# haoxiangsnr/Wave-U-Net-for-Speech-Enhancement

Hardware: AMD Instinct MI355X
Metric: 16384-sample frames/sec fwd+bwd, 12-level Wave-U-Net (higher is better)
Workload: dtype f32 (levels >= 16 samples: 3 x f16 MFMA on hi/lo fp16 halves, fp32 accumulate; the rest f32 MFMA); 1 GPU; unet_basic 12-level, 16384-sample frames, batch=64 per GPU, fp32, training-mode forward + smooth_l1 + backward + fused HIP Adam step (BASELINE.json configs[2]; configs[3] when n_gpus>1); global_batch=64, frame=16384, parallelism=dp1

## Files before the change

wave-u-net-for-speech-enhancement_amd/csrc/wunet_h3u.h:

```cpp
#pragma once
#include "wunet_h3.h"
#ifndef WUNET_H3U_ABL
#define WUNET_H3U_ABL 0
#endif

struct ConvH3uArgs {
    const float* z0; const float* a0; const float* s0;
    const float* z1; const float* a1; const float* s1;
    const float* xb0; const float* xb1;
    float* xsc;
    float up_scale;
    int Lt;
    int C0, C1, C8;
    const wunet_half* wh; unsigned wdelta;
    const float* bias; const float* sc2;
    float* out; float* stats;
    const float* ev_a; const float* ev_s; float* xrows;
    wunet_half* oxh; wunet_half* oxl;
    int B, Cout, L, logL, NS, ntiles, mblocks;
    unsigned long long* trace;
};

__device__ __forceinline__ void wunet_h3u_x_scale(const float* xb0, const float* xb1, float& s, float& inv)
{
    wunet_pow2_scale(fmaxf(xb0[0], xb1 ? xb1[0] : 0.0f), s, inv);
}

#define WUNET_H3U_NST 8
__device__ __forceinline__ void wunet_loader_barrier(int younger)
{
#ifdef WUNET_EMU
    (void)younger;
    emu::block_barrier();
#else
    if (younger >= 10 + WUNET_H3U_NST) asm volatile("s_waitcnt vmcnt(18) lgkmcnt(0)\n\ts_barrier" ::: "memory");
    else if (younger >= 10) asm volatile("s_waitcnt vmcnt(10) lgkmcnt(0)\n\ts_barrier" ::: "memory");
    else if (younger == 9) asm volatile("s_waitcnt vmcnt(9) lgkmcnt(0)\n\ts_barrier" ::: "memory");
    else asm volatile("s_waitcnt vmcnt(0) lgkmcnt(0)\n\ts_barrier" ::: "memory");
    wunet_sched_fence();
#endif
}

__device__ __forceinline__ void wunet_loader_stats_barrier(int younger)
{
#ifdef WUNET_EMU
    (void)younger;
    emu::block_barrier();
#else
    if (younger >= 10 + WUNET_H3U_NST) asm volatile("s_waitcnt lgkmcnt(0) vmcnt(18)\n\ts_barrier" ::: "memory");
    else if (younger >= 10) asm volatile("s_waitcnt lgkmcnt(0) vmcnt(10)\n\ts_barrier" ::: "memory");
    else asm volatile("s_waitcnt lgkmcnt(0) vmcnt(0)\n\ts_barrier" ::: "memory");
    wunet_sched_fence();
#endif
}

struct WunetH3uRaw { wunet_f4 q[8]; float ma, mb; };
struct WunetH3uTile { int b, l0, mt0, ch; };
struct WunetH3uCursor { int ch, tile, mb; };
struct WunetH3uStep { int NS, mblocks, qG, rG; };
__device__ __forceinline__ void wunet_h3u_advance(WunetH3uCursor& c, const WunetH3uStep& S)
{
    if (++c.ch == S.NS) {
        c.ch = 0; c.tile += S.qG; c.mb += S.rG;
        if (c.mb >= S.mblocks) { c.mb -= S.mblocks; ++c.tile; }
    }
}
struct WunetH3uCoord { float w0[4], w1[4], mw0, mw1; };
__device__ __forceinline__ void wunet_h3u_coord(const ConvH3uArgs& A, int l0, int lane, WunetH3uCoord& K)
{
    const int Lth = A.Lt >> 1, P = l0 - 2 + 4 * lane;
#pragma unroll
    for (int j = 0; j < 4; ++j) {
        int i0, i1;
        wunet_up_coord(P + j < 0 ? 0 : P + j, Lth, A.up_scale, i0, i1, K.w0[j], K.w1[j]);
    }
    const int p_m = l0 + 254 + (lane & 3);
    int i0, i1;
    wunet_up_coord((lane < 32 && p_m < A.Lt) ? p_m : 0, Lth, A.up_scale, i0, i1, K.mw0, K.mw1);
}
__device__ __forceinline__ void wunet_h3u_mini_src(const ConvH3uArgs& A, int l0, int lane, int& i0, int& i1)
{
    const int p_m = l0 + 254 + (lane & 3);
    float w0, w1;
    wunet_up_coord((lane < 32 && p_m < A.Lt) ? p_m : 0, A.Lt >> 1, A.up_scale, i0, i1, w0, w1);
}

__device__ __forceinline__ unsigned long long wunet_sgpr64(unsigned long long b)
{
#ifdef WUNET_EMU
    return b;
#else
    const unsigned blo = __builtin_amdgcn_readfirstlane((unsigned)b), bhi = __builtin_amdgcn_readfirstlane((unsigned)(b >> 32));
    return ((unsigned long long)bhi << 32) | blo;
#endif
}
__device__ __forceinline__ wunet_f4 wunet_ld4s_async(unsigned long long sbase, unsigned voff)
{
#ifdef WUNET_EMU
    wunet_f4 v;
    std::memcpy(&v, reinterpret_cast<const char*>(sbase) + voff, 16);
    return v;
#else
    wunet_f4 v;
    asm volatile("global_load_dwordx4 %0, %1, %2" : "=v"(v) : "v"(voff), "s"(sbase) : "memory");
    return v;
#endif
}
__device__ __forceinline__ float wunet_ld1s_async(unsigned long long sbase, unsigned voff)
{
#ifdef WUNET_EMU
    float v;
    std::memcpy(&v, reinterpret_cast<const char*>(sbase) + voff, 4);
    return v;
#else
    float v;
    asm volatile("global_load_dword %0, %1, %2" : "=v"(v) : "v"(voff), "s"(sbase) : "memory");
    return v;
#endif
}
template <int N>
__device__ __forceinline__ void wunet_vm_wait()
{
#ifndef WUNET_EMU
    asm volatile("s_waitcnt vmcnt(%0)" :: "n"(N) : "memory");
    wunet_sched_fence();
#endif
}
__device__ __forceinline__ unsigned wunet_m0_save()
{
#ifdef WUNET_EMU
    return 0;
#else
    unsigned keep;
    asm volatile("s_mov_b32 %0, m0" : "=s"(keep) :: "memory");
    return keep;
#endif
}
__device__ __forceinline__ void wunet_m0_restore(unsigned keep)
{
#ifndef WUNET_EMU
    asm volatile("s_mov_b32 m0, %0" :: "s"(keep) : "memory");
#else
    (void)keep;
#endif
}
#ifdef WUNET_EMU
#define wunet_lds_uniform(X_) (X_)
#else
#define wunet_lds_uniform(X_) ((unsigned)__builtin_amdgcn_readfirstlane((int)(X_)))
#endif
template <int IMM>
__device__ __forceinline__ void wunet_dma16m(unsigned long long sbase, unsigned voff, wunet_lds_t lds_base)
{
#ifdef WUNET_EMU
    wunet_dma16(reinterpret_cast<const char*>(sbase) + voff, lds_base + IMM);
#else
    asm volatile("s_add_u32 m0, %2, %3\n\ts_nop 0\n\tglobal_load_lds_dwordx4 %0, %1" :: "v"(voff), "s"(sbase), "s"(lds_base), "n"(IMM) : "memory", "scc");
#endif
}

__device__ __forceinline__ int wunet_h3u_issue(const ConvH3uArgs& A, WunetH3uRaw& R, const WunetH3uTile& T, int cw, int lane, int mi0, int mi1)
{
    if (WUNET_H3U_ABL & 1) return 0;
    const int c8 = wunet_uniform(T.ch * 4 + cw);
    const int L = A.L, Lh = L >> 1, Lth = A.Lt >> 1;
    const bool none = c8 >= A.C8, up = !none && c8 * 8 < A.C0;
    const int P = T.l0 - 2 + 4 * lane;
    const int e_m = (lane >> 2) & 7, p_m = T.l0 + 254 + (lane & 3);
    const bool in_m = lane < 32 && p_m < A.Lt;
    int wb = (T.l0 >> 1) - 2 + 2 * lane;
    wb = wb < 0 ? 0 : (wb > Lth - 4 ? Lth - 4 : wb);
    const int pc = P < 0 ? 0 : (P > L - 4 ? L - 4 : P);
    const unsigned rs = none ? 0u : up ? (unsigned)Lh : (unsigned)L;
    const float* const zrow = up ? A.z0 + ((size_t)T.b * A.C0 + c8 * 8) * Lh : none ? A.z1 : A.z1 + ((size_t)T.b * A.C1 + (c8 * 8 - A.C0)) * L;
    unsigned long long rb = wunet_sgpr64((unsigned long long)(__UINTPTR_TYPE__)zrow);
    const unsigned long long rb0 = rb;
    const unsigned voff = none ? 0u : (unsigned)(up ? wb : pc) * 4u;
    const int m0 = up ? mi0 : (in_m ? p_m : 0), m1 = up ? mi1 : m0;
#pragma unroll
    for (int e = 0; e < 8; ++e) {
        R.q[e] = wunet_ld4s_async(rb, voff);
        rb = wunet_sgpr64(rb + (unsigned long long)rs * 4u);
    }
    R.ma = wunet_ld1s_async(rb0, none ? 0u : ((unsigned)e_m * rs + (unsigned)m0) * 4u);
    R.mb = wunet_ld1s_async(rb0, none ? 0u : ((unsigned)e_m * rs + (unsigned)m1) * 4u);
    return 10;
}

template <bool EDGE, bool COPY>
__device__ __forceinline__ void wunet_h3u_convert_t(const ConvH3uArgs& A, const WunetH3uRaw& R, const WunetH3uTile& T, wunet_half* xs, int cw,
                                                    int lane, const WunetH3uCoord& K, const float* coef, unsigned long long* tr)
{
#ifdef WUNET_H3U_TRACE
#define WUNET_H3U_SUB(K_) if (tr && cw == 0 && lane == 0) tr[K_] = wunet_memtime();
#else
#define WUNET_H3U_SUB(K_)
    (void)tr;
#endif
    WUNET_H3U_SUB(0)
    constexpr int COLS = 272, Q4 = COLS / 4;
    if (WUNET_H3U_ABL & 16) return;
    if (WUNET_H3U_ABL & 64) {
        float t = R.ma + R.mb;
#pragma unroll
        for (int e = 0; e < 8; ++e) t += R.q[e][0] + R.q[e][1] + R.q[e][2] + R.q[e][3];
        if (t == 123.456f) xs[lane] = 1;
        return;
    }
    const int c8 = wunet_uniform(T.ch * 4 + cw);
    const int L = A.L;
    const bool none = c8 >= A.C8, up = !none && c8 * 8 < A.C0;
    if (none) {
        const wunet_h8 z{0, 0, 0, 0, 0, 0, 0, 0};
#pragma unroll
        for (int j = 0; j < 4; ++j) {
            const int col = 4 * lane + 6 + j;
            const int pw = (cw * COLS + (col & 3) * Q4 + (col >> 2)) * 8;
            wunet_sth8(xs + pw, z);
            wunet_sth8(xs + 4 * COLS * 8 + pw, z);
        }
        if (lane < 32) {
            const int col = 262 + (lane & 3);
            const int pw = (cw * COLS + (col & 3) * Q4 + (col >> 2)) * 8 + (lane >> 2);
            xs[pw] = 0;
            xs[4 * COLS * 8 + pw] = 0;
        }
        return;
    }
    const bool write_out = COPY && T.mt0 == 0;
    const int cc = c8 * 8;
    float av[8], sv[8];
#pragma unroll
    for (int e = 0; e < 8; ++e) { av[e] = coef[cc + e]; sv[e] = coef[A.C8 * 8 + cc + e]; }
    WUNET_H3U_SUB(1)
    const int P = T.l0 - 2 + 4 * lane;
    const bool edge = EDGE && P < 0;
    float vals[4][8];
    if (up) {
#pragma unroll
        for (int e = 0; e < 8; ++e) {
            float u[4];
#pragma unroll
            for (int k = 0; k < 4; ++k) u[k] = wunet_lrelu(av[e] * R.q[e][k] + sv[e]);
            const float t0 = u[0], t1 = edge ? u[0] : u[1], t2 = edge ? u[0] : u[2], t3 = edge ? u[1] : u[3];
            vals[0][e] = K.w0[0] * t0 + K.w1[0] * t1;
            vals[1][e] = K.w0[1] * t1 + K.w1[1] * t2;
            vals[2][e] = K.w0[2] * t1 + K.w1[2] * t2;
            vals[3][e] = K.w0[3] * t2 + K.w1[3] * t3;
        }
    } else {
#pragma unroll
        for (int e = 0; e < 8; ++e) {
            float u[4];
#pragma unroll
            for (int k = 0; k < 4; ++k) u[k] = wunet_lrelu(av[e] * R.q[e][k] + sv[e]);
            vals[0][e] = u[0]; vals[1][e] = u[1];
            vals[2][e] = edge ? u[0] : u[2];
            vals[3][e] = edge ? u[1] : u[3];
        }
    }
    WUNET_H3U_SUB(2)
#pragma unroll
    for (int j = 0; j < 4; ++j) {
        wunet_h8 h, l;
#pragma unroll
        for (int e = 0; e < 8; ++e) {
            wunet_half x, y;
            wunet_split_h((edge && j < 2) ? 0.0f : vals[j][e], x, y);
            wunet_put_half(h, e, x);
            wunet_put_half(l, e, y);
        }
        const int col = 4 * lane + 6 + j;
        const int pw = (cw * COLS + (col & 3) * Q4 + (col >> 2)) * 8;
        if (!(WUNET_H3U_ABL & 128) || h[0] == (wunet_half)0x1234) {
        wunet_sth8(xs + pw, h);
        wunet_sth8(xs + 4 * COLS * 8 + pw, l);
        }
        if (write_out && col >= 8 && col < 264) {
            const size_t o = (((size_t)T.b * A.C8 + c8) * L + (size_t)(P + j)) * 8;
            wunet_sth8(A.oxh + o, h);
            wunet_sth8(A.oxl + o, l);
        }
    }
    WUNET_H3U_SUB(3)
    if (lane < 32) {
        const int e_m = lane >> 2, p_m = T.l0 + 254 + (lane & 3);
        const bool in_m = p_m < A.Lt;
        const float am = coef[cc + e_m], sm = coef[A.C8 * 8 + cc + e_m];
        const float ua = wunet_lrelu(am * R.ma + sm);
        const float v = up ? K.mw0 * ua + K.mw1 * wunet_lrelu(am * R.mb + sm) : ua;
        wunet_half x, y;
        wunet_split_h(in_m ? v : 0.0f, x, y);
        const int col = 262 + (lane & 3);
        const int pw = (cw * COLS + (col & 3) * Q4 + (col >> 2)) * 8 + e_m;
        xs[pw] = x;
        xs[4 * COLS * 8 + pw] = y;
        if (write_out && col < 264) {
            const size_t o = (((size_t)T.b * A.C8 + c8) * L + (size_t)p_m) * 8 + e_m;
            A.oxh[o] = x;
            A.oxl[o] = y;
        }
    }
#undef WUNET_H3U_SUB
}
template <bool COPY>
__device__ __forceinline__ void wunet_h3u_convert(const ConvH3uArgs& A, const WunetH3uRaw& R, const WunetH3uTile& T, wunet_half* xs, int cw,
                                                  int lane, const WunetH3uCoord& K, const float* coef, unsigned long long* tr = nullptr)
{
    if (wunet_uniform(T.l0) == 0) wunet_h3u_convert_t<true, COPY>(A, R, T, xs, cw, lane, K, coef, tr);
    else wunet_h3u_convert_t<false, COPY>(A, R, T, xs, cw, lane, K, coef, tr);
}

#ifdef WUNET_H3U_TRACE
#define WUNET_H3U_SUBPTR (A.trace && t < 128 ? A.trace + 256 * 2 * 128 * 2 + ((size_t)blockIdx.x * 128 + t) * 4 : nullptr)
#define WUNET_H3U_STAMP(ROLE_, STAGE_, WHICH_)                                                                     \
    if (A.trace && cw == 0 && lane == 0 && (STAGE_) < 128)                                                         \
        A.trace[(((size_t)blockIdx.x * 2 + (ROLE_)) * 128 + (STAGE_)) * 2 + (WHICH_)] = wunet_memtime();
#else
#define WUNET_H3U_SUBPTR nullptr
#define WUNET_H3U_STAMP(ROLE_, STAGE_, WHICH_)
#endif

static_assert(10 + WUNET_H3U_NST == 18, "the barrier spellings above");
static_assert(20 + 2 * (2 * 4 + 1) + 2 * WUNET_H3U_NST <= 63, "vmcnt is a 6-bit field");
template <int M_REP, bool COPY = false>
__global__ __launch_bounds__(2 * WUNET_THREADS, 1) void conv_h3u_kernel(ConvH3uArgs A)
{
    constexpr int PAD = 2, TG = 5;
    constexpr int COLS = 272, Q4 = COLS / 4;
    constexpr int XP = 2 * 4 * COLS;
    constexpr int WPM = TG * 64;
    constexpr int WP = 2 * M_REP * WPM;
    static_assert(WPM == 320, "W run = 256 + 64 pieces");
    WUNET_DYN_SMEM(smem);
    wunet_half* const xs0 = reinterpret_cast<wunet_half*>(smem);
    wunet_half* const ws0 = xs0 + 2 * XP * 8;
    float* const red = reinterpret_cast<float*>(ws0 + 2 * WP * 8);
    float* const coef = red + WUNET_WAVES * M_REP * 32 + 4;
    const int ER = A.mblocks * M_REP * 16;
    float* const epi = coef + 2 * A.C8 * 8;

    const int tid = threadIdx.x, lane = tid & 63, wave = wunet_uniform(tid >> 6);
    const int cw = wave & 3;
    const int L = A.L;
    const int G = gridDim.x, nitems = A.ntiles * A.mblocks;
    if ((int)blockIdx.x >= nitems) return;
    const int nmy = (nitems - (int)blockIdx.x + G - 1) / G;
    const bool want_stats = A.stats != nullptr;

    float xs_ = 1.0f, xinv_ = 1.0f;
    wunet_h3u_x_scale(A.xb0, A.xb1, xs_, xinv_);
    if (blockIdx.x == 0 && tid == 0 && A.xsc) { A.xsc[0] = xs_; A.xsc[1] = xinv_; }

    for (int c = tid; c < A.C8 * 8; c += 2 * WUNET_THREADS) {
        const bool u = c < A.C0, k = c < A.C0 + A.C1;
        coef[c] = xs_ * (u ? A.a0[c] : k ? A.a1[c - A.C0] : 0.0f);
        coef[A.C8 * 8 + c] = xs_ * (u ? A.s0[c] : k ? A.s1[c - A.C0] : 0.0f);
    }
    for (int c = tid; c < ER; c += 2 * WUNET_THREADS) {
        const bool in = c < A.Cout;
        epi[c] = (in && A.bias) ? A.bias[c] : 0.0f;
        epi[ER + c] = (in && A.xrows) ? A.ev_a[c] : 0.0f;
        epi[2 * ER + c] = (in && A.xrows) ? A.ev_s[c] : 0.0f;
    }
    __syncthreads();
    if (wave >= WUNET_WAVES) {
        const wunet_lds_t ws_a = wunet_lds_addr(ws0);
        const unsigned wo_all = (unsigned)(cw * 64 + lane) * 16u, wo_rest = (256u + (unsigned)lane) * 16u;
        const int T = nmy * A.NS;
        const WunetH3uStep S{A.NS, A.mblocks, G / A.mblocks, G % A.mblocks};
#define WUNET_H3U_TILE(CUR_, OUT_)                                                                                 \
    WunetH3uTile OUT_;                                                                                             \
    OUT_.ch = (CUR_).ch; OUT_.mt0 = (CUR_).mb * M_REP;                                                             \
    OUT_.b = ((CUR_).tile * 256) >> A.logL; OUT_.l0 = ((CUR_).tile * 256) & (L - 1);
        const unsigned long long wrun = (unsigned long long)A.NS * (TG * 64 * 16);
#define WUNET_H3U_DMA_W(TL_, P_)                                                                                   \
    if (!(WUNET_H3U_ABL & 8)) {                                                                                    \
        const unsigned long long wb_ = (unsigned long long)(__UINTPTR_TYPE__)A.wh                                  \
                                     + (unsigned long long)((size_t)(TL_).mt0 * A.NS + (TL_).ch) * (TG * 64 * 16); \
        const wunet_lds_t la_ = ws_a + ((P_) * WP + cw * 64) * 16, lr_ = ws_a + ((P_) * WP + 256) * 16;            \
        const unsigned keep_ = wunet_m0_save();                                                                    \
        _Pragma("unroll") for (int sub = 0; sub < 2 * M_REP; ++sub) {                                              \
            const unsigned long long run_ = wunet_sgpr64(wb_ + (unsigned long long)(sub % M_REP) * wrun + (sub >= M_REP ? (unsigned long long)A.wdelta : 0ull)); \
            WUNET_H3U_DMA_PIECE(sub, run_, wo_all, la_)                                                            \
            if (cw == (sub & 3)) { WUNET_H3U_DMA_PIECE(sub, run_, wo_rest, lr_) }                                  \
        }                                                                                                          \
        wunet_m0_restore(keep_);                                                                                   \
    }
#define WUNET_H3U_DMA_PIECE(SUB_, RUN_, VOFF_, LB_)                                                                \
    switch (SUB_) {                                                                                                \
    case 0: wunet_dma16m<0 * WPM * 16>(RUN_, VOFF_, wunet_lds_uniform(LB_)); break;                                \
    case 1: wunet_dma16m<1 * WPM * 16>(RUN_, VOFF_, wunet_lds_uniform(LB_)); break;                                \
    case 2: wunet_dma16m<2 * WPM * 16>(RUN_, VOFF_, wunet_lds_uniform(LB_)); break;                                \
    case 3: wunet_dma16m<3 * WPM * 16>(RUN_, VOFF_, wunet_lds_uniform(LB_)); break;                                \
    case 4: wunet_dma16m<4 * WPM * 16>(RUN_, VOFF_, wunet_lds_uniform(LB_)); break;                                \
    case 5: wunet_dma16m<5 * WPM * 16>(RUN_, VOFF_, wunet_lds_uniform(LB_)); break;                                \
    case 6: wunet_dma16m<6 * WPM * 16>(RUN_, VOFF_, wunet_lds_uniform(LB_)); break;                                \
    default: wunet_dma16m<7 * WPM * 16>(RUN_, VOFF_, wunet_lds_uniform(LB_)); break;                               \
    }
        static_assert(M_REP <= 4, "eight runs per W sub-tile");
        WunetH3uRaw R0, R1, R2;
        int wo_p = 0, wo_pp = 0;
#define WUNET_H3U_COPIES(T_) ((COPY && (T_).mt0 == 0 && (T_).ch * 4 + cw < A.C8) ? 1 : 0)
        WunetH3uCursor c1, c3;
        int i3;
        WunetH3uCoord K;
        int mi0, mi1;
        {
            const int tile0 = (int)blockIdx.x / A.mblocks;
            c1 = WunetH3uCursor{0, tile0, (int)blockIdx.x - tile0 * A.mblocks};
            WUNET_H3U_TILE(c1, t0)
            c3 = c1; i3 = 0;
            if (T > 1) { wunet_h3u_advance(c3, S); ++i3; }
            WUNET_H3U_TILE(c3, t1)
            wunet_h3u_coord(A, t0.l0, lane, K);
            wunet_h3u_mini_src(A, t0.l0, lane, mi0, mi1);
            wunet_h3u_issue(A, R0, t0, cw, lane, mi0, mi1);
            if (t1.ch == 0) wunet_h3u_mini_src(A, t1.l0, lane, mi0, mi1);
            wunet_h3u_issue(A, R1, t1, cw, lane, mi0, mi1);
            WUNET_H3U_DMA_W(t0, 0)
            if (T > 2) { wunet_h3u_advance(c3, S); ++i3; }
            WUNET_H3U_TILE(c3, t2)
            if (t2.ch == 0) wunet_h3u_mini_src(A, t2.l0, lane, mi0, mi1);
            wunet_h3u_issue(A, R2, t2, cw, lane, mi0, mi1);
            wunet_vm_wait<0>();
            wunet_h3u_convert<COPY>(A, R0, t0, xs0, cw, lane, K, coef);
            wo_p = WUNET_H3U_COPIES(t0);
        }
#define WUNET_H3U_LOADER_STAGE(CUR_, FREE_)                                                                        \
    {                                                                                                              \
        WUNET_H3U_STAMP(1, t, 0)                                                                                   \
        if (COPY) wunet_loader_barrier((WUNET_H3U_ABL & 1) ? 0 : 10 + wo_p * WUNET_H3U_NST);                       \
        else wunet_loader_barrier((WUNET_H3U_ABL & 1) ? 0 : 10);              \
        WUNET_H3U_STAMP(1, t, 1)                                                                                   \
        wunet_h3u_advance(c1, S);                                                                                  \
        WUNET_H3U_TILE(c1, tn)                                                                                     \
        WUNET_H3U_DMA_W(tn, (t + 1) & 1)                                                                           \
        if (i3 < T - 1) { wunet_h3u_advance(c3, S); ++i3; }                                                        \
        WUNET_H3U_TILE(c3, tnn)                                                                                    \
        if (tnn.ch == 0) wunet_h3u_mini_src(A, tnn.l0, lane, mi0, mi1);                                            \
        wunet_h3u_issue(A, FREE_, tnn, cw, lane, mi0, mi1);                                                        \
        if (tn.ch == 0) wunet_h3u_coord(A, tn.l0, lane, K);                                                        \
         \
        if (COPY) {                                                                                                \
            const int nwo_ = wunet_uniform(wo_p + wo_pp);                                                          \
            if (nwo_ == 0) wunet_vm_wait<20 + 2 * (2 * M_REP + 1)>();                                              \
            else if (nwo_ == 1) wunet_vm_wait<20 + 2 * (2 * M_REP + 1) + WUNET_H3U_NST>();                         \
            else wunet_vm_wait<20 + 2 * (2 * M_REP + 1) + 2 * WUNET_H3U_NST>();                                    \
        } else wunet_vm_wait<20 + 2 * (2 * M_REP + 1)>();                                                          \
        wunet_h3u_convert<COPY>(A, CUR_, tn, xs0 + ((t + 1) & 1) * XP * 8, cw, lane, K, coef, WUNET_H3U_SUBPTR);    \
        if (COPY) { wo_pp = wo_p; wo_p = WUNET_H3U_COPIES(tn); }                                                   \
        if (want_stats && tn.ch == 0) wunet_loader_stats_barrier((WUNET_H3U_ABL & 1) ? 0 : 10 + wo_p * WUNET_H3U_NST); \
        ++t;                                                                                                       \
    }
        int t = 0;
        while (t < T - 1) {
            WUNET_H3U_LOADER_STAGE(R1, R0)
            if (t >= T - 1) break;
            WUNET_H3U_LOADER_STAGE(R2, R1)
            if (t >= T - 1) break;
            WUNET_H3U_LOADER_STAGE(R0, R2)
        }
        wunet_loader_barrier(0);
        if (want_stats) wunet_loader_stats_barrier(0);
#undef WUNET_H3U_LOADER_STAGE
#undef WUNET_H3U_COPIES
#undef WUNET_H3U_DMA_W
#undef WUNET_H3U_DMA_PIECE
#undef WUNET_H3U_TILE
        return;
    }

    const int q = lane >> 4, i16 = lane & 15;
    const int ll0 = cw * 64 + i16 * 4;
    const int boff = (q * COLS + (ll0 >> 2)) * 8;
    const int aoff = (q * 16 + i16) * 8;
    int par = 0;
    float amax_run = 0.0f;
    const float inv12 = xinv_ * (A.sc2 ? A.sc2[1] : 1.0f);
    for (int k = 0; k < nmy; ++k) {
        const int v = (int)blockIdx.x + k * G, tile = v / A.mblocks, mblk = v - tile * A.mblocks;
        const int b = (tile * 256) >> A.logL, l0 = (tile * 256) & (L - 1), mt0 = mblk * M_REP;
        wunet_f4 acc[M_REP][4];
#pragma unroll
        for (int mt = 0; mt < M_REP; ++mt)
#pragma unroll
            for (int nt = 0; nt < 4; ++nt) acc[mt][nt] = wunet_f4{0.f, 0.f, 0.f, 0.f};
        for (int st = 0; st < A.NS; ++st) {
            WUNET_H3U_STAMP(0, k * A.NS + st, 0)
            wunet_wait_lds_barrier();
            WUNET_H3U_STAMP(0, k * A.NS + st, 1)
            if (WUNET_H3U_ABL & 32) { par ^= 1; continue; }
            const wunet_half* const xs = xs0 + par * XP * 8;
            const wunet_half* const ws = ws0 + par * WP * 8;
            wunet_h8 fh[TG + 3], fl[TG + 3];
#pragma unroll
            for (int e = 0; e < TG + 3; ++e) {
                const int ec = e + 8 - PAD;
                const int po = ((ec & 3) * Q4 + (ec >> 2)) * 8;
                fh[e] = wunet_ldh8(xs + boff + po);
                fl[e] = wunet_ldh8(xs + 4 * COLS * 8 + boff + po);
            }
            wunet_h8 ah[2][M_REP], al[2][M_REP];
#define WUNET_H3U_LOAD_A(BUF_, TL_)                                                                               \
    _Pragma("unroll") for (int mt = 0; mt < M_REP; ++mt) {                                                        \
        ah[BUF_][mt] = wunet_ldh8(ws + ((mt * TG + (TL_)) * 64) * 8 + aoff);                                      \
        al[BUF_][mt] = wunet_ldh8(ws + ((M_REP + mt) * TG + (TL_)) * 64 * 8 + aoff);                              \
    }
#define WUNET_H3U_PASS(WHICH_, BUF_, TL_)                                                                         \
    _Pragma("unroll") for (int mt = 0; mt < M_REP; ++mt)                                                          \
        _Pragma("unroll") for (int nt = 0; nt < 4; ++nt) {                                                        \
            if (WUNET_H3U_ABL & 4) { if ((WHICH_) == 0 && (TL_) == 0) acc[mt][nt][0] += (float)al[BUF_][mt][0] + (float)fh[nt][0] + (float)ah[BUF_][mt][1] + (float)fl[nt][1]; } \
            else if ((WHICH_) == 0) acc[mt][nt] = wunet_mfma16h(al[BUF_][mt], fh[(TL_) + nt], acc[mt][nt]);       \
            else if ((WHICH_) == 1) acc[mt][nt] = wunet_mfma16h(ah[BUF_][mt], fl[(TL_) + nt], acc[mt][nt]);       \
            else acc[mt][nt] = wunet_mfma16h(ah[BUF_][mt], fh[(TL_) + nt], acc[mt][nt]);                          \
        }
#define WUNET_H3U_STEP(TL_)                                                                                       \
    {                                                                                                             \
        constexpr int tl = (TL_);                                                                                 \
        if (tl + 1 < TG) {                                                                                        \
            if (tl & 1) { WUNET_H3U_LOAD_A(0, tl + 1) } else { WUNET_H3U_LOAD_A(1, tl + 1) }                      \
        }                                                                                                         \
        wunet_sched_fence();                                                                                      \
        if (tl & 1) { WUNET_H3U_PASS(0, 1, tl) WUNET_H3U_PASS(1, 1, tl) WUNET_H3U_PASS(2, 1, tl) }               \
        else { WUNET_H3U_PASS(0, 0, tl) WUNET_H3U_PASS(1, 0, tl) WUNET_H3U_PASS(2, 0, tl) }                      \
    }
            WUNET_H3U_LOAD_A(0, 0)
            WUNET_H3U_STEP(0) WUNET_H3U_STEP(1) WUNET_H3U_STEP(2) WUNET_H3U_STEP(3) WUNET_H3U_STEP(4)
#undef WUNET_H3U_STEP
#undef WUNET_H3U_PASS
#undef WUNET_H3U_LOAD_A
            par ^= 1;
        }

        {
            float amax = 0.0f;
            float bvs[M_REP][4];
#pragma unroll
            for (int mt = 0; mt < M_REP; ++mt)
#pragma unroll
                for (int r = 0; r < 4; ++r) bvs[mt][r] = epi[(mt0 + mt) * 16 + q * 4 + r];
            float* const prow = A.out + ((size_t)b * A.Cout + mt0 * 16 + q * 4) * L + (l0 + ll0);
            const bool full = (mt0 + M_REP) * 16 <= A.Cout;
#define WUNET_H3U_ROWS(STATS_, GUARD_, EVAL_)                                                                     \
    float eas[M_REP][4], ess[M_REP][4];                                                                           \
    if (EVAL_) {                                                                                                  \
        _Pragma("unroll") for (int mt = 0; mt < M_REP; ++mt)                                                      \
            _Pragma("unroll") for (int r = 0; r < 4; ++r) {                                                       \
                const int co = (mt0 + mt) * 16 + q * 4 + r;                                                       \
                eas[mt][r] = epi[ER + co];                                                                        \
                ess[mt][r] = epi[2 * ER + co];                                                                    \
            }                                                                                                     \
    }                                                                                                             \
    _Pragma("unroll") for (int mt = 0; mt < M_REP; ++mt) {                                                        \
        float s1[4] = {0.f, 0.f, 0.f, 0.f}, s2[4] = {0.f, 0.f, 0.f, 0.f};                                         \
        _Pragma("unroll") for (int r = 0; r < 4; ++r) {                                                           \
            const int co = (mt0 + mt) * 16 + q * 4 + r;                                                           \
            const float bv = bvs[mt][r];                                                                          \
            wunet_f4 o;                                                                                           \
            _Pragma("unroll") for (int nt = 0; nt < 4; ++nt) {                                                    \
                const float vv = acc[mt][nt][r] * inv12;                                                          \
                if (STATS_) { s1[r] += vv; s2[r] = fmaf(vv, vv, s2[r]); }                                         \
                o[nt] = vv + bv;                                                                                  \
            }                                                                                                     \
            if (!(GUARD_) || co < A.Cout) {                                                                       \
                wunet_st4(prow + (size_t)(mt * 16 + r) * L, o);                                                   \
                if (EVAL_) {                                                                                      \
                    const float ea = eas[mt][r], es = ess[mt][r];                                                 \
                    _Pragma("unroll") for (int nt = 0; nt < 4; ++nt) amax = fmaxf(amax, fabsf(ea * o[nt] + es));  \
                }                                                                                                 \
            }                                                                                                     \
        }                                                                                                         \
        if (STATS_) {                                                                                             \
            _Pragma("unroll") for (int r = 0; r < 4; ++r) {                                                       \
                s1[r] = wunet_row16_sum(s1[r]);                                                                   \
                s2[r] = wunet_row16_sum(s2[r]);                                                                   \
                if (i16 == 0) {                                                                                   \
                    float* rp = red + ((cw * M_REP + mt) * 16 + q * 4 + r) * 2;                                   \
                    rp[0] = s1[r];                                                                                \
                    rp[1] = s2[r];                                                                                \
                }                                                                                                 \
            }                                                                                                     \
        }                                                                                                         \
    }
            if (A.xrows) { WUNET_H3U_ROWS(false, true, true) }
            else if (want_stats) { if (full) { WUNET_H3U_ROWS(true, false, false) } else { WUNET_H3U_ROWS(true, true, false) } }
            else { if (full) { WUNET_H3U_ROWS(false, false, false) } else { WUNET_H3U_ROWS(false, true, false) } }
#undef WUNET_H3U_ROWS
            if (A.xrows) {
#pragma unroll
                for (int m = 1; m < 64; m <<= 1) amax = fmaxf(amax, wunet_shfl_xor(amax, m));
                amax_run = fmaxf(amax_run, amax);
            }
        }
        if (want_stats) {
            wunet_wait_lds_barrier();
            if (tid < M_REP * 16) {
                const float* rp = red + tid * 2;
                float t1 = 0.0f, t2 = 0.0f;
#pragma unroll
                for (int w = 0; w < WUNET_WAVES; ++w) {
                    t1 += rp[w * M_REP * 32];
                    t2 += rp[w * M_REP * 32 + 1];
                }
                const int co = mt0 * 16 + tid;
                if (co < A.Cout) {
                    float* stp = A.stats + ((size_t)co * A.ntiles + tile) * 2;
                    stp[0] = t1;
                    stp[1] = t2;
                }
            }
        }
    }
    if (A.xrows && lane == 0) wunet_atomic_absmax(A.xrows, amax_run);
}
```

Before: 12790 frames/s.

## Move converted-input copy-out stores from loader waves to MFMA consumer waves

The global copy of the fp16 hi/lo converted input (oxh/oxl) is no longer written by the loader waves during conversion. It is now stored by the compute waves from the fragments they already read out of LDS, interleaved between MFMA steps. This removes the extra vmcnt bookkeeping and deeper waits the loader needed to track those stores, which shortens the loader's critical path. The cost is extra global stores in the MFMA loop, where they may contend with matrix work, and a copy layout that now depends on the consumer's fragment mapping.

```diff
diff --git a/wave-u-net-for-speech-enhancement_amd/csrc/wunet_h3u.h b/wave-u-net-for-speech-enhancement_amd/csrc/wunet_h3u.h
--- a/wave-u-net-for-speech-enhancement_amd/csrc/wunet_h3u.h
+++ b/wave-u-net-for-speech-enhancement_amd/csrc/wunet_h3u.h
@@ -26,15 +26,13 @@
     wunet_pow2_scale(fmaxf(xb0[0], xb1 ? xb1[0] : 0.0f), s, inv);
 }
 
-#define WUNET_H3U_NST 8
 __device__ __forceinline__ void wunet_loader_barrier(int younger)
 {
 #ifdef WUNET_EMU
     (void)younger;
     emu::block_barrier();
 #else
-    if (younger >= 10 + WUNET_H3U_NST) asm volatile("s_waitcnt vmcnt(18) lgkmcnt(0)\n\ts_barrier" ::: "memory");
-    else if (younger >= 10) asm volatile("s_waitcnt vmcnt(10) lgkmcnt(0)\n\ts_barrier" ::: "memory");
+    if (younger >= 10) asm volatile("s_waitcnt vmcnt(10) lgkmcnt(0)\n\ts_barrier" ::: "memory");
     else if (younger == 9) asm volatile("s_waitcnt vmcnt(9) lgkmcnt(0)\n\ts_barrier" ::: "memory");
     else asm volatile("s_waitcnt vmcnt(0) lgkmcnt(0)\n\ts_barrier" ::: "memory");
     wunet_sched_fence();
@@ -47,8 +45,7 @@
     (void)younger;
     emu::block_barrier();
 #else
-    if (younger >= 10 + WUNET_H3U_NST) asm volatile("s_waitcnt lgkmcnt(0) vmcnt(18)\n\ts_barrier" ::: "memory");
-    else if (younger >= 10) asm volatile("s_waitcnt lgkmcnt(0) vmcnt(10)\n\ts_barrier" ::: "memory");
+    if (younger >= 10) asm volatile("s_waitcnt lgkmcnt(0) vmcnt(10)\n\ts_barrier" ::: "memory");
     else asm volatile("s_waitcnt lgkmcnt(0) vmcnt(0)\n\ts_barrier" ::: "memory");
     wunet_sched_fence();
 #endif
@@ -187,7 +184,7 @@
     return 10;
 }
 
-template <bool EDGE, bool COPY>
+template <bool EDGE>
 __device__ __forceinline__ void wunet_h3u_convert_t(const ConvH3uArgs& A, const WunetH3uRaw& R, const WunetH3uTile& T, wunet_half* xs, int cw,
                                                     int lane, const WunetH3uCoord& K, const float* coef, unsigned long long* tr)
 {
@@ -208,7 +205,6 @@
         return;
     }
     const int c8 = wunet_uniform(T.ch * 4 + cw);
-    const int L = A.L;
     const bool none = c8 >= A.C8, up = !none && c8 * 8 < A.C0;
     if (none) {
         const wunet_h8 z{0, 0, 0, 0, 0, 0, 0, 0};
@@ -227,7 +223,6 @@
         }
         return;
     }
-    const bool write_out = COPY && T.mt0 == 0;
     const int cc = c8 * 8;
     float av[8], sv[8];
 #pragma unroll
@@ -275,11 +270,6 @@
         if (!(WUNET_H3U_ABL & 128) || h[0] == (wunet_half)0x1234) {
         wunet_sth8(xs + pw, h);
         wunet_sth8(xs + 4 * COLS * 8 + pw, l);
-        }
-        if (write_out && col >= 8 && col < 264) {
-            const size_t o = (((size_t)T.b * A.C8 + c8) * L + (size_t)(P + j)) * 8;
-            wunet_sth8(A.oxh + o, h);
-            wunet_sth8(A.oxl + o, l);
         }
     }
     WUNET_H3U_SUB(3)
@@ -295,20 +285,14 @@
         const int pw = (cw * COLS + (col & 3) * Q4 + (col >> 2)) * 8 + e_m;
         xs[pw] = x;
         xs[4 * COLS * 8 + pw] = y;
-        if (write_out && col < 264) {
-            const size_t o = (((size_t)T.b * A.C8 + c8) * L + (size_t)p_m) * 8 + e_m;
-            A.oxh[o] = x;
-            A.oxl[o] = y;
-        }
     }
 #undef WUNET_H3U_SUB
 }
-template <bool COPY>
 __device__ __forceinline__ void wunet_h3u_convert(const ConvH3uArgs& A, const WunetH3uRaw& R, const WunetH3uTile& T, wunet_half* xs, int cw,
                                                   int lane, const WunetH3uCoord& K, const float* coef, unsigned long long* tr = nullptr)
 {
-    if (wunet_uniform(T.l0) == 0) wunet_h3u_convert_t<true, COPY>(A, R, T, xs, cw, lane, K, coef, tr);
-    else wunet_h3u_convert_t<false, COPY>(A, R, T, xs, cw, lane, K, coef, tr);
+    if (wunet_uniform(T.l0) == 0) wunet_h3u_convert_t<true>(A, R, T, xs, cw, lane, K, coef, tr);
+    else wunet_h3u_convert_t<false>(A, R, T, xs, cw, lane, K, coef, tr);
 }
 
 #ifdef WUNET_H3U_TRACE
@@ -321,12 +305,12 @@
 #define WUNET_H3U_STAMP(ROLE_, STAGE_, WHICH_)
 #endif
 
-static_assert(10 + WUNET_H3U_NST == 18, "the barrier spellings above");
-static_assert(20 + 2 * (2 * 4 + 1) + 2 * WUNET_H3U_NST <= 63, "vmcnt is a 6-bit field");
+static_assert(20 + 2 * (2 * 4 + 1) <= 63, "vmcnt is a 6-bit field");
 template <int M_REP, bool COPY = false>
 __global__ __launch_bounds__(2 * WUNET_THREADS, 1) void conv_h3u_kernel(ConvH3uArgs A)
 {
     constexpr int PAD = 2, TG = 5;
+    static_assert(TG == 2 * PAD + 1, "one stage per channel chunk");
     constexpr int COLS = 272, Q4 = COLS / 4;
     constexpr int XP = 2 * 4 * COLS;
     constexpr int WPM = TG * 64;
@@ -400,8 +384,6 @@
     }
         static_assert(M_REP <= 4, "eight runs per W sub-tile");
         WunetH3uRaw R0, R1, R2;
-        int wo_p = 0, wo_pp = 0;
-#define WUNET_H3U_COPIES(T_) ((COPY && (T_).mt0 == 0 && (T_).ch * 4 + cw < A.C8) ? 1 : 0)
         WunetH3uCursor c1, c3;
         int i3;
         WunetH3uCoord K;
@@ -424,14 +406,12 @@
             if (t2.ch == 0) wunet_h3u_mini_src(A, t2.l0, lane, mi0, mi1);
             wunet_h3u_issue(A, R2, t2, cw, lane, mi0, mi1);
             wunet_vm_wait<0>();
-            wunet_h3u_convert<COPY>(A, R0, t0, xs0, cw, lane, K, coef);
-            wo_p = WUNET_H3U_COPIES(t0);
+            wunet_h3u_convert(A, R0, t0, xs0, cw, lane, K, coef);
         }
 #define WUNET_H3U_LOADER_STAGE(CUR_, FREE_)                                                                        \
     {                                                                                                              \
         WUNET_H3U_STAMP(1, t, 0)                                                                                   \
-        if (COPY) wunet_loader_barrier((WUNET_H3U_ABL & 1) ? 0 : 10 + wo_p * WUNET_H3U_NST);                       \
-        else wunet_loader_barrier((WUNET_H3U_ABL & 1) ? 0 : 10);              \
+        wunet_loader_barrier((WUNET_H3U_ABL & 1) ? 0 : 10);                                                        \
         WUNET_H3U_STAMP(1, t, 1)                                                                                   \
         wunet_h3u_advance(c1, S);                                                                                  \
         WUNET_H3U_TILE(c1, tn)                                                                                     \
@@ -441,16 +421,10 @@
         if (tnn.ch == 0) wunet_h3u_mini_src(A, tnn.l0, lane, mi0, mi1);                                            \
         wunet_h3u_issue(A, FREE_, tnn, cw, lane, mi0, mi1);                                                        \
         if (tn.ch == 0) wunet_h3u_coord(A, tn.l0, lane, K);                                                        \
-         \
-        if (COPY) {                                                                                                \
-            const int nwo_ = wunet_uniform(wo_p + wo_pp);                                                          \
-            if (nwo_ == 0) wunet_vm_wait<20 + 2 * (2 * M_REP + 1)>();                                              \
-            else if (nwo_ == 1) wunet_vm_wait<20 + 2 * (2 * M_REP + 1) + WUNET_H3U_NST>();                         \
-            else wunet_vm_wait<20 + 2 * (2 * M_REP + 1) + 2 * WUNET_H3U_NST>();                                    \
-        } else wunet_vm_wait<20 + 2 * (2 * M_REP + 1)>();                                                          \
-        wunet_h3u_convert<COPY>(A, CUR_, tn, xs0 + ((t + 1) & 1) * XP * 8, cw, lane, K, coef, WUNET_H3U_SUBPTR);    \
-        if (COPY) { wo_pp = wo_p; wo_p = WUNET_H3U_COPIES(tn); }                                                   \
-        if (want_stats && tn.ch == 0) wunet_loader_stats_barrier((WUNET_H3U_ABL & 1) ? 0 : 10 + wo_p * WUNET_H3U_NST); \
+                                                                   \
+        wunet_vm_wait<20 + 2 * (2 * M_REP + 1)>();                                                                 \
+        wunet_h3u_convert(A, CUR_, tn, xs0 + ((t + 1) & 1) * XP * 8, cw, lane, K, coef, WUNET_H3U_SUBPTR);         \
+        if (want_stats && tn.ch == 0) wunet_loader_stats_barrier((WUNET_H3U_ABL & 1) ? 0 : 10);                    \
         ++t;                                                                                                       \
     }
         int t = 0;
@@ -464,7 +438,6 @@
         wunet_loader_barrier(0);
         if (want_stats) wunet_loader_stats_barrier(0);
 #undef WUNET_H3U_LOADER_STAGE
-#undef WUNET_H3U_COPIES
 #undef WUNET_H3U_DMA_W
 #undef WUNET_H3U_DMA_PIECE
 #undef WUNET_H3U_TILE
@@ -486,6 +459,8 @@
         for (int mt = 0; mt < M_REP; ++mt)
 #pragma unroll
             for (int nt = 0; nt < 4; ++nt) acc[mt][nt] = wunet_f4{0.f, 0.f, 0.f, 0.f};
+        const bool copy_out = COPY && mt0 == 0;
+        const size_t cp_o = (((size_t)b * A.C8 + q) * L + (size_t)(l0 + ll0)) * 8, cp_st = (size_t)4 * L * 8;
         for (int st = 0; st < A.NS; ++st) {
             WUNET_H3U_STAMP(0, k * A.NS + st, 0)
             wunet_wait_lds_barrier();
@@ -501,6 +476,12 @@
                 fh[e] = wunet_ldh8(xs + boff + po);
                 fl[e] = wunet_ldh8(xs + 4 * COLS * 8 + boff + po);
             }
+            const bool copy_st = copy_out && st * 4 + q < A.C8;
+#define WUNET_H3U_COPY_OUT(J_)                                                                                    \
+    if (COPY && copy_st) {                                                                                        \
+        wunet_sth8(A.oxh + cp_o + (size_t)st * cp_st + (J_) * 8, fh[PAD + (J_)]);                                 \
+        wunet_sth8(A.oxl + cp_o + (size_t)st * cp_st + (J_) * 8, fl[PAD + (J_)]);                                 \
+    }
             wunet_h8 ah[2][M_REP], al[2][M_REP];
 #define WUNET_H3U_LOAD_A(BUF_, TL_)                                                                               \
     _Pragma("unroll") for (int mt = 0; mt < M_REP; ++mt) {                                                        \
@@ -526,7 +507,9 @@
         else { WUNET_H3U_PASS(0, 0, tl) WUNET_H3U_PASS(1, 0, tl) WUNET_H3U_PASS(2, 0, tl) }                      \
     }
             WUNET_H3U_LOAD_A(0, 0)
-            WUNET_H3U_STEP(0) WUNET_H3U_STEP(1) WUNET_H3U_STEP(2) WUNET_H3U_STEP(3) WUNET_H3U_STEP(4)
+            WUNET_H3U_STEP(0) WUNET_H3U_COPY_OUT(0) WUNET_H3U_STEP(1) WUNET_H3U_COPY_OUT(1) WUNET_H3U_STEP(2) WUNET_H3U_COPY_OUT(2)
+            WUNET_H3U_STEP(3) WUNET_H3U_COPY_OUT(3) WUNET_H3U_STEP(4)
+#undef WUNET_H3U_COPY_OUT
 #undef WUNET_H3U_STEP
 #undef WUNET_H3U_PASS
 #undef WUNET_H3U_LOAD_A
```

Measured after the change: 12660 frames/s. About the same (-1.0%).
